# davidmhunt/mmwave_radar_processing

Hardware: AMD Instinct MI355X
Metric: radar frames/s on 256×128×12 ADC cube, 1/2/4/8 GPU; % HBM roofline (higher is better)
Workload: dtype f32; 1 GPU; IWR1843 synthetic 256x128x(4Rx x 3Tx) cube: Hann range FFT + Doppler FFT + 64-bin angle FFT -> complex64 [64,256,128] (BASELINE configs[1]); frames_per_gpu=1250, angle_bins=64, arch=gfx950:sramecc+:xnack-, compute_units=256

## Files before the change

mmwave_radar_processing_amd/csrc/mmw_cells64.h:

```cpp
#pragma once
#include "mmw_ctx.h"
#include "mmw_misc.h"
#include "mmw_bf16x3.h"

namespace mmw {

struct Cells64Args {
    const float2 *cubes;
    const int32_t *dets;
    const int32_t *counts;
    const int *flagpos;
    const int *n_flag;
    int dense_min;
    cplx<double> *out;
    int V, S, cap, n_ant, max_cells;
    AntList ants;
    const double *ws, *wc;
    const cplx<double> *twS, *twC;
};

constexpr int C64_NT = 512, C64_ROWS = 64, C64_PITCH = 137, C64_CELLS = 256, C64_ITEMS = 8 * C64_CELLS / C64_NT;
inline size_t cells64_lds(int S, int C, int) {
    return ((size_t)C64_ROWS * C64_PITCH + S) * 16 + ((size_t)S + C) * 8 + (size_t)C64_CELLS * 8 + 64;
}
inline int cells64_max_cells(int S, int C) {
    return C == 128 && cells64_lds(S, C, 0) <= 160 * 1024 - 512 ? C64_CELLS : 0;
}

template <int C>
__global__ __launch_bounds__(C64_NT) void k_cells64(Cells64Args a) {
    static_assert(C == 128, "one Doppler row = 8 lanes x 16 points");
    constexpr int P = C64_PITCH;
    extern __shared__ __attribute__((aligned(16))) char smem[];
    if (*a.n_flag < a.dense_min) return;
    const int S = a.S, tid = threadIdx.x, lane = tid & 63, wave = tid >> 6, n1 = tid & 7, rl = tid >> 3;
    cplx<double> *Z = reinterpret_cast<cplx<double> *>(smem);
    cplx<double> *twS = Z + C64_ROWS * P;
    double *wsl = reinterpret_cast<double *>(twS + S), *wcl = wsl + S;
    int *cell_rk = reinterpret_cast<int *>(wcl + C), *cell_e = cell_rk + C64_CELLS, *wcnt = cell_e + C64_CELLS;
    const long f = blockIdx.y;
    const int ai = blockIdx.x;
    int n_det = a.counts[f];
    if (n_det > a.cap) n_det = a.cap;
    if (n_det <= 0) return;
    for (int i = tid; i < S; i += C64_NT) {
        twS[i] = a.twS[i];
        wsl[i] = a.ws[i];
    }
    for (int i = tid; i < C; i += C64_NT) wcl[i] = a.wc[i];
    cplx<double> tw1[16];
#pragma unroll
    for (int k2 = 1; k2 < 16; ++k2) tw1[k2] = a.twC[(n1 * k2) & (C - 1)];
    const float2 *plane = a.cubes + (f * a.V + a.ants.idx[ai]) * (long)S * C;
    cplx<double> *slab = Z + rl * P;
    for (int c0 = 0;; c0 += C64_CELLS) {
        int running = 0;
        for (int det0 = 0; det0 < n_det; det0 += C64_NT) {
            const int det = det0 + tid;
            const int e = det < n_det ? a.flagpos[f * a.cap + det] - 1 : -1;
            const unsigned long long bal = __ballot(e >= 0);
            if (lane == 0) wcnt[wave] = __popcll(bal);
            __syncthreads();
            int before = running, total = running;
#pragma unroll
            for (int w = 0; w < C64_NT / 64; ++w) {
                const int cw = wcnt[w];
                if (w < wave) before += cw;
                total += cw;
            }
            const int ord = before + __popcll(bal & ((1ull << lane) - 1ull)) - c0;
            if (e >= 0 && ord >= 0 && ord < C64_CELLS) {
                const int r = a.dets[(f * a.cap + det) * 2];
                int k = a.dets[(f * a.cap + det) * 2 + 1] - C / 2;
                if (k < 0) k += C;
                cell_rk[ord] = (r << 16) | k;
                cell_e[ord] = e;
            }
            running = total;
            __syncthreads();
        }
        const int n_cells = running - c0 < C64_CELLS ? running - c0 : C64_CELLS;
        if (n_cells <= 0) break;
        cplx<double> acc[C64_ITEMS];
#pragma unroll
        for (int j = 0; j < C64_ITEMS; ++j) acc[j] = cplx<double>{0.0, 0.0};
        float2 raw[16];
        auto fetch = [&](int s0) {
            const int s = s0 + rl, sc = s < S ? s : S - 1;
            const float2 *rowp = plane + (long)sc * C;
#pragma unroll
            for (int n2 = 0; n2 < 16; ++n2) raw[n2] = rowp[n1 + 8 * n2];
        };
        fetch(0);
        for (int s0 = 0; s0 < S; s0 += C64_ROWS) {
            {
                const int s = s0 + rl;
                const double wrow = s < S ? wsl[s] : 0.0;
                cplx<double> x[16];
#pragma unroll
                for (int n2 = 0; n2 < 16; ++n2) {
                    const double w = wcl[n1 + 8 * n2] * wrow;
                    x[n2] = cplx<double>{(double)raw[n2].x * w, (double)raw[n2].y * w};
                }
                fetch(s0 + C64_ROWS < S ? s0 + C64_ROWS : s0);
                RegFFT<16, double>::run(x);
                static_for<16>([&](auto K) {
                    constexpr int k2 = decltype(K)::value;
                    const cplx<double> v = x[bitrev<16>(k2)];
                    slab[k2 * 8 + ((n1 + k2) & 7)] = k2 == 0 ? v : cmul(v, tw1[k2]);
                });
                __builtin_amdgcn_wave_barrier();
                cplx<double> ya[8], yb[8];
#pragma unroll
                for (int n = 0; n < 8; ++n) {
                    ya[n] = slab[n1 * 8 + ((n + n1) & 7)];
                    yb[n] = slab[(n1 + 8) * 8 + ((n + n1) & 7)];
                }
                RegFFT<8, double>::run(ya);
                RegFFT<8, double>::run(yb);
                __builtin_amdgcn_wave_barrier();
                static_for<8>([&](auto K) {
                    constexpr int k1 = decltype(K)::value;
                    slab[n1 + 16 * k1] = ya[bitrev<8>(k1)];
                    slab[n1 + 8 + 16 * k1] = yb[bitrev<8>(k1)];
                });
            }
            __syncthreads();
#pragma unroll
            for (int j = 0; j < C64_ITEMS; ++j) {
                const int it = tid + j * C64_NT, i = it >> 3, q = it & 7;
                if (i < n_cells) {
                    const int rk = cell_rk[i], r = rk >> 16, k = rk & 0xffff;
                    const int sq = s0 + 8 * q;
                    cplx<double> c = twS[(int)(((long)r * sq) % S)];
                    const cplx<double> step = twS[r % S];
                    const cplx<double> *zp = Z + (8 * q) * P + k;
                    cplx<double> sum = acc[j];
#pragma unroll
                    for (int t = 0; t < 8; ++t) {
                        const cplx<double> z = zp[t * P];
                        sum.x = fma(z.x, c.x, fma(-z.y, c.y, sum.x));
                        sum.y = fma(z.x, c.y, fma(z.y, c.x, sum.y));
                        c = cmul(c, step);
                    }
                    acc[j] = sum;
                }
            }
            __syncthreads();
        }
#pragma unroll
        for (int j = 0; j < C64_ITEMS; ++j) {
            const int it = tid + j * C64_NT, i = it >> 3, q = it & 7;
            cplx<double> s = acc[j];
            for (int d = 1; d < 8; d <<= 1) {
                s.x += __shfl_xor(s.x, d, 64);
                s.y += __shfl_xor(s.y, d, 64);
            }
            if (i < n_cells && q == 0) a.out[(long)cell_e[i] * a.n_ant + ai] = s;
        }
        if (running <= c0 + C64_CELLS) break;
        __syncthreads();
    }
}

struct Rd64Args {
    const float2 *cubes;
    long frame_stride;
    double *mag;
    cplx<double> *scratch;
    int n_frames;
    const double *ws, *wc;
    const cplx<double> *twS, *twC;
};
constexpr int R64_S = 256, R64_C = 128, R64_COLS = 32, R64_CP = 257;
inline size_t rd64_lds() { return (std::max((size_t)C64_ROWS * C64_PITCH, (size_t)R64_COLS * R64_CP) + R64_S + R64_C) * 16 + (R64_S + R64_C) * 8; }

__global__ __launch_bounds__(C64_NT) void k_rd_mag64_256x128(Rd64Args a) {
    constexpr int S = R64_S, C = R64_C, P = C64_PITCH;
    extern __shared__ __attribute__((aligned(16))) char smem[];
    const int tid = threadIdx.x;
    cplx<double> *Z = reinterpret_cast<cplx<double> *>(smem);
    cplx<double> *twl = Z + (C64_ROWS * P > R64_COLS * R64_CP ? C64_ROWS * P : R64_COLS * R64_CP);
    cplx<double> *twc = twl + S;
    double *wsl = reinterpret_cast<double *>(twc + C), *wcl = wsl + S;
    for (int i = tid; i < S; i += C64_NT) {
        wsl[i] = a.ws[i];
        twl[i] = a.twS[i];
    }
    for (int i = tid; i < C; i += C64_NT) {
        wcl[i] = a.wc[i];
        twc[i] = a.twC[i];
    }
    cplx<double> *T = a.scratch + (size_t)blockIdx.x * S * C;
    const auto t_rs = __builtin_amdgcn_make_buffer_rsrc(T, 0, S * C * 16, 0x00020000);
    __syncthreads();
    for (long f = blockIdx.x; f < a.n_frames; f += gridDim.x) {
        const float2 *plane = a.cubes + f * a.frame_stride;
        {
            const int n1 = tid & 7, rl = tid >> 3;
            cplx<double> *slab = Z + rl * P;
            float2 raw[16];
            auto fetch = [&](int s0) {
                const float2 *rowp = plane + (long)(s0 + rl) * C;
#pragma unroll
                for (int n2 = 0; n2 < 16; ++n2) raw[n2] = rowp[n1 + 8 * n2];
            };
            fetch(0);
            for (int s0 = 0; s0 < S; s0 += C64_ROWS) {
                const double wrow = wsl[s0 + rl];
                cplx<double> x[16];
#pragma unroll
                for (int n2 = 0; n2 < 16; ++n2) {
                    const double w = wcl[n1 + 8 * n2] * wrow;
                    x[n2] = cplx<double>{(double)raw[n2].x * w, (double)raw[n2].y * w};
                }
                fetch(s0 + C64_ROWS < S ? s0 + C64_ROWS : s0);
                RegFFT<16, double>::run(x);
                static_for<16>([&](auto K) {
                    constexpr int k2 = decltype(K)::value;
                    const cplx<double> v = x[bitrev<16>(k2)];
                    slab[k2 * 8 + ((n1 + k2) & 7)] = k2 == 0 ? v : cmul(v, twc[(n1 * k2) & (C - 1)]);
                });
                __builtin_amdgcn_wave_barrier();
                cplx<double> ya[8], yb[8];
#pragma unroll
                for (int n = 0; n < 8; ++n) {
                    ya[n] = slab[n1 * 8 + ((n + n1) & 7)];
                    yb[n] = slab[(n1 + 8) * 8 + ((n + n1) & 7)];
                }
                RegFFT<8, double>::run(ya);
                RegFFT<8, double>::run(yb);
                __builtin_amdgcn_wave_barrier();
                static_for<8>([&](auto K) {
                    constexpr int k1 = decltype(K)::value;
                    slab[n1 + 16 * k1] = ya[bitrev<8>(k1)];
                    slab[n1 + 8 + 16 * k1] = yb[bitrev<8>(k1)];
                });
                __syncthreads();
#pragma unroll 4
                for (int i = tid; i < C * C64_ROWS; i += C64_NT) {
                    const int k = i >> 6, r = i & 63;
                    T[k * S + s0 + r] = Z[r * P + k];
                }
                __syncthreads();
            }
        }
        asm volatile("s_waitcnt vmcnt(0)" ::: "memory");
        __syncthreads();
        {
            const int m1 = tid & 15, cl = tid >> 4;
            cplx<double> *slab = Z + cl * R64_CP;
            double *out = a.mag + f * (long)S * C;
            for (int k0 = 0; k0 < C; k0 += R64_COLS) {
                const int k = k0 + cl;
                cplx<double> x[16];
#pragma unroll
                for (int m2 = 0; m2 < 16; ++m2) {
                    const u32x4 v = __builtin_bit_cast(u32x4, __builtin_amdgcn_raw_buffer_load_b128(t_rs, (unsigned)((k * S + m1 + 16 * m2) * 16), 0, 1));
                    x[m2] = __builtin_bit_cast(cplx<double>, v);
                }
                RegFFT<16, double>::run(x);
                static_for<16>([&](auto Q) {
                    constexpr int q = decltype(Q)::value;
                    const cplx<double> v = x[bitrev<16>(q)];
                    slab[q * 16 + ((m1 + q) & 15)] = q == 0 ? v : cmul(v, twl[(m1 * q) & (S - 1)]);
                });
                __builtin_amdgcn_wave_barrier();
                cplx<double> y[16];
#pragma unroll
                for (int n = 0; n < 16; ++n) y[n] = slab[m1 * 16 + ((n + m1) & 15)];
                RegFFT<16, double>::run(y);
                int d = k + C / 2;
                if (d >= C) d -= C;
                static_for<16>([&](auto Pp) {
                    constexpr int p = decltype(Pp)::value;
                    const cplx<double> v = y[bitrev<16>(p)];
                    out[(long)(m1 + 16 * p) * C + d] = hypot(v.x, v.y);
                });
                __builtin_amdgcn_wave_barrier();
            }
        }
        __syncthreads();
    }
}

struct Argmax64ListArgs {
    const cplx<double> *cells;
    const int *n_flag, *list;
    int dense_min, dense_cap, n_ant, A, shift;
    int32_t *out_idx;
    const cplx<double> *twA;
};
__global__ __launch_bounds__(256) void k_argmax64_list(Argmax64ListArgs a) {
    int n = *a.n_flag;
    if (n < a.dense_min) return;
    if (n > a.dense_cap) n = a.dense_cap;
    const int lane = threadIdx.x & 63;
    for (int e = blockIdx.x * 4 + (threadIdx.x >> 6); e < n; e += gridDim.x * 4) {
        const int idx = argmax64_wave(a.cells + (long)e * a.n_ant, a.n_ant, a.A, a.shift, a.twA, lane);
        if (lane == 0) a.out_idx[a.list[e] & 0x7fffffff] = idx;
    }
}

}
```

mmwave_radar_processing_amd/csrc/mmw_cfar.h:

```cpp
#pragma once
#include "mmw_ctx.h"

namespace mmw {

template <int DEPTH, typename G> __device__ double np_pairwise(G get, int lo, int n) {
    if (n < 8) {
        double res = 0.0;
        for (int i = 0; i < n; ++i) res += get(lo + i);
        return res;
    }
    if (n <= 128 || DEPTH == 0) {
        double r0 = get(lo + 0), r1 = get(lo + 1), r2 = get(lo + 2), r3 = get(lo + 3);
        double r4 = get(lo + 4), r5 = get(lo + 5), r6 = get(lo + 6), r7 = get(lo + 7);
        int i = 8;
        for (; i < n - (n % 8); i += 8) {
            r0 += get(lo + i + 0); r1 += get(lo + i + 1); r2 += get(lo + i + 2); r3 += get(lo + i + 3);
            r4 += get(lo + i + 4); r5 += get(lo + i + 5); r6 += get(lo + i + 6); r7 += get(lo + i + 7);
        }
        double res = ((r0 + r1) + (r2 + r3)) + ((r4 + r5) + (r6 + r7));
        for (; i < n; ++i) res += get(lo + i);
        return res;
    }
    if constexpr (DEPTH > 0) {
        int n2 = n / 2;
// ... 567 lines not shown
    const double *base = tile + (ty * OSV_NV) * TW + tx;
#pragma unroll 1
    for (int y = 0; y < WR + OSV_NV - 1; ++y) {
        double v[WD];
#pragma unroll
        for (int wd = 0; wd < WD; ++wd) v[wd] = base[y * TW + wd];
        static_for<OSV_NV>([&](auto J) {
            constexpr int j = decltype(J)::value;
            const int wr = y - j;
            if (wr >= 0 && wr < WR) {
                if (wr >= TR && wr <= TR + 2 * GR) {
                    static_for<WD>([&](auto Wd) {
                        constexpr int wd = decltype(Wd)::value;
                        if constexpr (wd < TD || wd > TD + 2 * GD) below[j] += v[wd] < x[j] ? 1 : 0;
                    });
                } else {
#pragma unroll
                    for (int wd = 0; wd < WD; ++wd) below[j] += v[wd] < x[j] ? 1 : 0;
                }
            }
        });
    }
#pragma unroll
    for (int j = 0; j < OSV_NV; ++j) {
        const int r = rb + j;
        if (r >= p.R) break;
        const bool valid = r >= HR && r < p.R - HR && c >= HD && c < p.D - HD;
        p.mask[(long)blockIdx.z * plane + (long)r * p.D + c] = (valid && below[j] >= p.k_rank) ? 1 : 0;
    }
}

struct Cfar1dArgs {
    const double *x;
    double *thr, *noise;
    uint8_t *mask;
    int n_rows, L;
    int kind, T, G;
    double scale;
    int k_rank;
};

__device__ __forceinline__ double cfar1d_threshold(const Cfar1dArgs &p, const double *x, int i, double *est_out) {
    const int half = p.T + p.G;
    double thr = INFINITY, est = 0.0;
    if (i >= half && i < p.L - half) {
        const double *w = x + (i - half);
        const int rs = p.T + 2 * p.G + 1;
        if (p.kind == MMW_CFAR_CA) {
            double s = 0.0;
            if (p.L == 2 * half + 1) {
                s = np_pairwise<3>([&](int q) { return q < p.T ? w[q] : w[rs + q - p.T]; }, 0, 2 * p.T);
            } else {
                for (int q = 0; q < p.T; ++q) s += w[q];
                for (int q = 0; q < p.T; ++q) s += w[rs + q];
            }
            est = s / (double)(2 * p.T);
        } else if (p.kind == MMW_CFAR_OS) {
            est = kth_smallest([&](int q) { return q < p.T ? w[q] : w[rs + q - p.T]; }, 2 * p.T, p.k_rank);
        } else {
            const double ml = np_pairwise<2>([&](int q) { return w[q]; }, 0, p.T) / (double)p.T;
            const double mr = np_pairwise<2>([&](int q) { return w[rs + q]; }, 0, p.T) / (double)p.T;
            est = (ml != ml || mr != mr) ? ml + mr : (p.kind == MMW_CFAR_GO) ? fmax(ml, mr) : fmin(ml, mr);
        }
        thr = p.scale * est;
    }
    *est_out = est;
    return thr;
}

__global__ __launch_bounds__(256) void k_cfar1d(Cfar1dArgs p) {
    const long gid = (long)blockIdx.x * 256 + threadIdx.x;
    if (gid >= (long)p.n_rows * p.L) return;
    const int i = (int)(gid % p.L);
    const double *x = p.x + (gid - i);
    double est;
    const double thr = cfar1d_threshold(p, x, i, &est);
    if (p.thr) p.thr[gid] = thr;
    if (p.noise) p.noise[gid] = est;
    if (p.mask) p.mask[gid] = (x[i] > thr) ? 1 : 0;
}

__global__ __launch_bounds__(1024) void k_compact2d(const uint8_t *mask, int32_t *dets, int32_t *counts,
                                                    int R, int D, int cap) {
    __shared__ int wave_tot[16];
    __shared__ int wave_off[16];
    const long cells = (long)R * D;
    const uint8_t *m = mask + (long)blockIdx.x * cells;
    const int per = (int)((cells + 1023) / 1024);
    const long lo = (long)threadIdx.x * per;
    const long hi = lo + per < cells ? lo + per : cells;
    int cnt = 0;
    for (long i = lo; i < hi; ++i) cnt += m[i] ? 1 : 0;
    const int lane = threadIdx.x & 63, wave = threadIdx.x >> 6;
    int incl = cnt;
    for (int d = 1; d < 64; d <<= 1) {
        const int v = __shfl_up(incl, d, 64);
        if (lane >= d) incl += v;
    }
    if (lane == 63) wave_tot[wave] = incl;
    __syncthreads();
    if (threadIdx.x == 0) {
        int run = 0;
        for (int w = 0; w < 16; ++w) {
            wave_off[w] = run;
            run += wave_tot[w];
        }
        counts[blockIdx.x] = run;
    }
    __syncthreads();
    int pos = wave_off[wave] + incl - cnt;
    int32_t *out = dets + (long)blockIdx.x * cap * 2;
    for (long i = lo; i < hi; ++i) {
        if (m[i]) {
            if (pos < cap) {
                out[2 * pos] = (int32_t)(i / D);
                out[2 * pos + 1] = (int32_t)(i % D);
            }
            ++pos;
        }
    }
}

}
```

mmwave_radar_processing_amd/csrc/mmwgpu.hip:

```cpp
#include "mmw_ctx.h"
#include "mmw_launch.h"
#include "mmw_cfar.h"
#include "mmw_ground.h"
#include "mmw_seq.h"
#include "mmw_misc.h"
#include "mmw_czt.h"
#include "mmw_beamform.h"
#include "mmw_detect.h"
#include "mmw_cells64.h"

#include <algorithm>
#include <climits>
#include <chrono>
#include <memory>
#include <cstdlib>
#include <thread>

using namespace mmw;

namespace {

int env_int(const char *name, int dflt) {
    const char *s = std::getenv(name);
    return (s && *s) ? std::atoi(s) : dflt;
// ... 417 lines not shown
    MMW_REQUIRE(ctx && d_cubes && d_out, "null argument");
    MMW_REQUIRE(n_frames >= 0 && V > 0 && S > 0 && C > 0, "bad shape");
    if (n_frames == 0) return MMW_OK;
    {
        ProfScope ps(ctx, "rd");
        bool l1_done = false;
        const bool i16_folded = rv.i16 && rv.ntx > 1 &&
                                (fused_rd_runs(S, C) ||
                                 (rd_mixed_ct_supported(S, C) && !env_int("MMW_NO_MIXED_RD", 0)));
        if (rv.i16 && !i16_folded) {
            MMW_REQUIRE(rv.ntx >= 1 && rv.nrx >= 1, "int16 cubes are raw cubes");
            const long total = (long)n_frames * V * S * C;
            hipLaunchKernelGGL(k_reformat_i16, dim3((unsigned)((total + 255) / 256)), dim3(256), 0, ctx->stream,
                               (const short2 *)d_cubes, (float2 *)d_out, total, rv.nrx, rv.ntx, S, C);
            MMW_TRY(check_launch("reformat_i16"));
            d_cubes = d_out;
            rv = RawView{1, 0, rv.vskip, 0};
        }
        if (fused_rd_runs(S, C))
            MMW_TRY(launch_rd_fused(ctx, d_cubes, d_out, n_frames * V, S, C, rv, rv.ntx > 1 ? nullptr : d_l1, &l1_done));
        else if (rd_lds_supported(S, C) && !env_int("MMW_NO_FUSED_RD", 0) && !rd_mixed_ct_supported(S, C))
            MMW_TRY(launch_rd_lds(ctx, d_cubes, d_out, n_frames * V, S, C, rv));
        else if (rd_mixed_ct_supported(S, C) && !env_int("MMW_NO_MIXED_RD", 0)) {
            float *l1 = rv.ntx > 1 ? nullptr : d_l1;
            MMW_TRY(launch_rd_mixed_ct(ctx, d_cubes, (long)S * C, d_out, n_frames * V, S, C, rv, nullptr, 0, nullptr, false, l1));
            l1_done = l1 != nullptr;
        } else if (rd_mixed_supported(S, C) && !env_int("MMW_NO_MIXED_RD", 0))
            MMW_TRY((launch_rd_mixed<float, false>(ctx, d_cubes, (long)S * C, d_out, n_frames * V, S, C, rv)));
        else if (rv.ntx <= 1 && rd_split_ct_supported(S, C) && !env_int("MMW_NO_SPLIT_RD", 0))
            MMW_TRY(launch_rd_split_ct(ctx, d_cubes, d_out, n_frames * V, S, C, rv));
        else if (rv.ntx > 1) {
            const long total = (long)n_frames * V * S * C;
            hipLaunchKernelGGL(k_reformat, dim3((unsigned)((total + 255) / 256)), dim3(256), 0, ctx->stream,
                               (const float2 *)d_cubes, (float2 *)d_out, total, rv.nrx, rv.ntx, S, C);
            MMW_TRY(check_launch("reformat"));
            if (rd_split_ct_supported(S, C) && !env_int("MMW_NO_SPLIT_RD", 0))
                MMW_TRY(launch_rd_split_ct(ctx, d_out, d_out, n_frames * V, S, C, RawView{1, 0, rv.vskip}));
            else
                MMW_TRY(range_doppler_generic(ctx, d_out, d_out, n_frames, V, S, C));
        } else
            MMW_TRY(range_doppler_generic(ctx, d_cubes, d_out, n_frames, V, S, C));
        if (d_l1 && !l1_done) {
            MMW_REQUIRE(rv.ntx <= 1, "plane L1 norms are defined on virtual-array cubes");
            MMW_TRY(plane_l1_impl(ctx, d_cubes, d_l1, n_frames, V, S, C));
        }
    }
    if (d_mag_f32) MMW_TRY(abs_c64(ctx, d_out, (float *)d_mag_f32, (size_t)n_frames * V * S * C));
    return MMW_OK;
}

int mmw_range_doppler(mmw_ctx *ctx, const void *d_cubes, void *d_out, void *d_mag_f32, int n_frames, int V,
                      int S, int C) {
    MMW_REQUIRE(ctx, "ctx is null");
    MMW_JOIN(ctx);
    return range_doppler_impl(ctx, d_cubes, d_out, d_mag_f32, n_frames, V, S, C);
}

static int range_doppler_mag64_impl(mmw_ctx *ctx, const void *d_cubes, double *d_mag, int n_frames, int V, int S,
                                   int C, int rx_idx) {
    MMW_REQUIRE(ctx && d_cubes && d_mag, "null argument");
    MMW_REQUIRE(n_frames >= 0 && V > 0 && S > 0 && C > 0 && rx_idx >= 0 && rx_idx < V, "bad shape / rx_idx");
    if (n_frames == 0) return MMW_OK;
    ProfScope ps(ctx, "rd64");
    if (S == R64_S && C == R64_C && n_frames >= 8 && opt_int(ctx, "MMW_RD64_FUSED", 1)) {
        const int grid = std::min(n_frames, ctx->num_cu);
        MMW_TRY(ensure_scratch(ctx, (size_t)grid * S * C * sizeof(cplx<double>)));
        Rd64Args ra{};
        ra.cubes = (const float2 *)d_cubes + (long)rx_idx * S * C;
        ra.frame_stride = (long)V * S * C;
        ra.mag = d_mag;
        ra.scratch = (cplx<double> *)ctx->scratch;
        ra.n_frames = n_frames;
        const void *p;
        MMW_TRY(get_table<double>(ctx, TAB_HANN, S, &p));
        ra.ws = (const double *)p;
        MMW_TRY(get_table<double>(ctx, TAB_HANN, C, &p));
        ra.wc = (const double *)p;
        MMW_TRY(get_table<double>(ctx, TAB_TWIDDLE, S, &p));
        ra.twS = (const cplx<double> *)p;
        MMW_TRY(get_table<double>(ctx, TAB_TWIDDLE, C, &p));
        ra.twC = (const cplx<double> *)p;
        const size_t lds = rd64_lds();
        MMW_HIP(hipFuncSetAttribute(reinterpret_cast<const void *>(k_rd_mag64_256x128), hipFuncAttributeMaxDynamicSharedMemorySize, (int)lds));
        hipLaunchKernelGGL(k_rd_mag64_256x128, dim3((unsigned)grid), dim3(C64_NT), lds, ctx->stream, ra);
        return check_launch("rd_mag64_256x128");
    }
    RdMixedPlan mp;
    if (!is_pow2(S) || !is_pow2(C) || (long)S * C >= 8192)
        if (rd_mixed_plan(S, C, sizeof(cplx<double>), &mp) && !env_int("MMW_NO_MIXED_RD", 0))
            return launch_rd_mixed<double, true>(ctx, (const cplx<float> *)d_cubes + (long)rx_idx * S * C,
                                                 (long)V * S * C, d_mag, n_frames, S, C);
    const size_t plane_bytes = (size_t)S * C * sizeof(cplx<double>);
    long chunk = (long)(((size_t)128 << 20) / plane_bytes);
    if (chunk < 1) chunk = 1;
    if (chunk > n_frames) chunk = n_frames;
    MMW_TRY(ensure_scratch(ctx, (size_t)chunk * plane_bytes));
    FftArgs a{};
    a.out = ctx->scratch;
    a.inner = C;
    a.n_in = S;
    a.in_outer_stride = (long)V * S * C;
    a.out_outer_stride = (long)S * C;
    a.in_axis_stride = a.out_axis_stride = C;
    a.in_inner_stride = a.out_inner_stride = 1;
    MMW_TRY(get_table<double>(ctx, TAB_HANN, S, &a.win_axis));
    MMW_TRY(get_table<double>(ctx, TAB_HANN, C, &a.win_inner));
    a.scale = 1.0;
    FftArgs b{};
    b.in = ctx->scratch;
    b.inner = 1;
    b.n_in = C;
    b.in_outer_stride = b.out_outer_stride = C;
    b.in_axis_stride = b.out_axis_stride = 1;
    b.scale = 1.0;
    b.shift = 1;
    b.magnitude = 1;
    for (long f0 = 0; f0 < n_frames; f0 += chunk) {
        const int nf = (int)std::min<long>(chunk, n_frames - f0);
        a.in = (const cplx<float> *)d_cubes + (f0 * V + rx_idx) * (long)S * C;
        a.outer = nf;
        MMW_TRY((launch_fft_axis<double, float>(ctx, a, S, false)));
        b.out = d_mag + f0 * (long)S * C;
        b.outer = nf * S;
        MMW_TRY((launch_fft_axis<double, double>(ctx, b, C, true)));
    }
    return MMW_OK;
}

int mmw_range_doppler_mag64(mmw_ctx *ctx, const void *d_cubes, double *d_mag, int n_frames, int V, int S,
                            int C, int rx_idx) {
    MMW_REQUIRE(ctx, "ctx is null");
    MMW_JOIN(ctx);
    return range_doppler_mag64_impl(ctx, d_cubes, d_mag, n_frames, V, S, C, rx_idx);
}

static bool angle_fast_path(int V, long bins, int A, bool mag);

static int angle_fft_impl(mmw_ctx *ctx, const void *d_rd, void *d_out, int n_frames, int V, int S, int C, int A,
                         int flags) {
    MMW_REQUIRE(ctx && d_rd && d_out, "null argument");
    MMW_REQUIRE(n_frames >= 0 && V > 0 && S > 0 && C > 0 && A >= V, "bad shape (need A >= V)");
    MMW_REQUIRE((flags & ~7) == 0, "unknown flag bits %d", flags);
    if (n_frames == 0) return MMW_OK;
    const bool magnitude = flags & MMW_ANGLE_MAGNITUDE, window = !(flags & MMW_ANGLE_NO_WINDOW),
               shift = !(flags & MMW_ANGLE_NO_SHIFT);
    ProfScope ps(ctx, "angle");
    const long bins = (long)S * C;
    if (n_frames <= 65535 && angle_fast_path(V, bins, A, magnitude)) {
        float h[16];
        for (int i = 0; i < V; ++i) h[i] = window ? (float)np_window(TAB_HANN, i, V) : 1.f;
        switch (V) {
            case 4: return launch_angle64<4>(ctx, d_rd, d_out, n_frames, bins, magnitude, h, shift);
            case 8: return launch_angle64<8>(ctx, d_rd, d_out, n_frames, bins, magnitude, h, shift);
            case 12: return launch_angle64<12>(ctx, d_rd, d_out, n_frames, bins, magnitude, h, shift);
            default: return launch_angle64<16>(ctx, d_rd, d_out, n_frames, bins, magnitude, h, shift);
        }
    }
    FftArgs a{};
    a.in = d_rd;
    a.out = d_out;
    a.outer = n_frames;
    a.inner = (int)bins;
    a.n_in = V;
    a.in_outer_stride = (long)V * bins;
    a.out_outer_stride = (long)A * bins;
    a.in_axis_stride = a.out_axis_stride = bins;
    a.in_inner_stride = a.out_inner_stride = 1;
// ... 1098 lines not shown
    if (!no_mixed && rd_mixed_plan(S, C, sizeof(cplx<float>), &mp))
        return structured + mp.s1 + mp.s2 + mp.c1 + mp.c2 + 2 * (mp.rad_s[0] + mp.rad_s[1] + mp.rad_c[0] + mp.rad_c[1]);
    if (rd_split_ct_supported(S, C) && !env_int("MMW_NO_SPLIT_RD", 0)) return structured;
    int ulps = 8;
    for (int axis = 0; axis < 2; ++axis) {
        const int n = axis ? C : S;
        if (is_pow2(n)) ulps += 4 * ilog2(n);
        else ulps += n + 4;
    }
    return ulps;
}

static int launch_argmax_refine(mmw_ctx *ctx, const RefineArgs &ra) {
    const size_t lds = refine_tabs_lds(ra.S, ra.C);
    MMW_REQUIRE(lds <= 150 * 1024, "plane %d x %d too large for the refinement tables", ra.S, ra.C);
    if (lds > 48 * 1024) {
        MMW_HIP(hipFuncSetAttribute(reinterpret_cast<const void *>(k_argmax_refine_part), hipFuncAttributeMaxDynamicSharedMemorySize, (int)lds));
        MMW_HIP(hipFuncSetAttribute(reinterpret_cast<const void *>(k_argmax_refine_whole), hipFuncAttributeMaxDynamicSharedMemorySize, (int)lds));
    }
    if (ra.n_split > 0) {
        const int units = std::min(ra.n_split, std::max(1, 512));
        hipLaunchKernelGGL(k_argmax_refine_part, dim3(ra.parts, units), dim3(256), lds, ctx->stream, ra);
        MMW_TRY(check_launch("argmax_refine_part"));
        hipLaunchKernelGGL(k_argmax_refine_finish, dim3(std::min((ra.n_split + 3) / 4, ctx->num_cu)), dim3(256), 0, ctx->stream, ra);
        MMW_TRY(check_launch("argmax_refine_finish"));
    }
    if (ra.list_cap > ra.n_split) {
        hipLaunchKernelGGL(k_argmax_refine_whole, dim3(ctx->num_cu), dim3(256), lds, ctx->stream, ra);
        MMW_TRY(check_launch("argmax_refine_whole"));
    }
    return MMW_OK;
}

static int refine_parts(int n_frames) {
    int p = REFINE_PARTS;
    while (p > 2 && (long)p * n_frames > 60000) p /= 2;
    return p;
}

static int fill_refine_args(mmw_ctx *ctx, RefineArgs *ra, const void *d_cubes, const int32_t *d_dets, const int *n_flag, const int *list,
                            int list_cap, int n_split, cplx<double> *partial, int n_frames, int V, int S, int C, int cap, int A) {
    ra->cubes = (const float2 *)d_cubes, ra->dets = d_dets, ra->V = V, ra->cap = cap;
    ra->n_flag = n_flag, ra->list = list, ra->list_cap = list_cap;
    ra->partial = partial, ra->n_split = n_split, ra->parts = refine_parts(n_frames);
    const void *twA64, *twS64, *twC64, *ws64, *wc64;
    MMW_TRY(get_table<double>(ctx, TAB_TWIDDLE, A, &twA64));
    MMW_TRY(get_table<double>(ctx, TAB_TWIDDLE, S, &twS64));
    MMW_TRY(get_table<double>(ctx, TAB_TWIDDLE, C, &twC64));
    MMW_TRY(get_table<double>(ctx, TAB_HANN, S, &ws64));
    MMW_TRY(get_table<double>(ctx, TAB_HANN, C, &wc64));
    ra->S = S;
    ra->C = C;
    ra->A = A;
    ra->ws = (const double *)ws64;
    ra->wc = (const double *)wc64;
    ra->twS = (const cplx<double> *)twS64;
    ra->twC = (const cplx<double> *)twC64;
    ra->twA = (const cplx<double> *)twA64;
    return MMW_OK;
}

static float argmax_bound_div(const mmw_ctx *ctx) { return (float)std::max(1, opt_int(ctx, "MMW_ARGMAX_BOUND_DIV", 1)); }


int mmw_angle_argmax_exact(mmw_ctx *ctx, const void *d_cubes, const float *d_l1, const void *d_rd, const int32_t *d_dets,
                           const int32_t *d_counts, int32_t *d_idx, int n_frames, int V, int S, int C, int cap,
                           const int *h_ant, int n_ant, int A, int shift, int *h_n_refined) {
    MMW_REQUIRE(ctx && d_cubes && d_l1 && d_rd && d_dets && d_counts && d_idx, "null argument");
    MMW_JOIN(ctx);
    MMW_REQUIRE(n_frames >= 0 && n_frames <= 65535 && V > 0 && S > 0 && C > 0 && cap >= 0 && A > 0, "bad shape");
    MMW_REQUIRE((long)n_frames * cap < (1L << 31), "too many detection slots for one call");
    AntList ants{};
    MMW_TRY(fill_ant_list(h_ant, n_ant, V, A, &ants));
    if (h_n_refined) *h_n_refined = 0;
    if (n_frames == 0 || cap == 0) return MMW_OK;
    const void *twA = nullptr;
    MMW_TRY(get_table<float>(ctx, TAB_TWIDDLE, A, &twA));
    const int list_cap = n_frames * cap;
    const int n_split = std::min(list_cap, std::max(0, opt_int(ctx, "MMW_REFINE_SPLIT", 32768)));
    const int max_cells = C == 128 ? cells64_max_cells(S, C) : 0;
    const int dense_min = max_cells > 0 ? std::max(1, opt_int(ctx, "MMW_ARGMAX_DENSE_MIN", 8 * n_frames)) : 0;
    const int dense_cap = dense_min > 0 ? (int)std::min<long>(list_cap, 256L * n_frames) : 0;
    auto up = [](size_t b) { return (b + 255) & ~(size_t)255; };
    const size_t list_bytes = up(256 + (size_t)list_cap * sizeof(int));
    const size_t part_bytes = up((size_t)n_split * REFINE_PARTS * n_ant * sizeof(cplx<double>));
    const size_t pos_bytes = dense_min > 0 ? up((size_t)list_cap * sizeof(int)) : 0;
    const size_t cell_bytes = up((size_t)dense_cap * n_ant * sizeof(cplx<double>));
    MMW_TRY(ensure_scratch(ctx, list_bytes + part_bytes + pos_bytes + cell_bytes));
    int *d_nflag = (int *)ctx->scratch, *d_list = (int *)((char *)ctx->scratch + 256);
    int *d_flagpos = dense_min > 0 ? (int *)((char *)ctx->scratch + list_bytes + part_bytes) : nullptr;
    cplx<double> *d_cells = (cplx<double> *)((char *)ctx->scratch + list_bytes + part_bytes + pos_bytes);
    MMW_HIP(hipMemsetAsync(d_nflag, 0, 256, ctx->stream));
    if (d_flagpos) MMW_HIP(hipMemsetAsync(d_flagpos, 0, (size_t)list_cap * sizeof(int), ctx->stream));
    const float eps = 5.9604645e-8f, div = argmax_bound_div(ctx);
    ArgmaxRefine rf{d_l1, d_nflag, d_list, list_cap, (float)rd_error_ulps(S, C) * eps / div, 4.f * (float)(n_ant + 4) * eps / div,
                    d_flagpos, dense_cap};
    ProfScope ps(ctx, "argmax");
    dim3 grid(std::min((cap + 3) / 4, 32), n_frames);
    launch_angle_argmax(ctx, grid, (const float2 *)d_rd, d_dets, d_counts, d_idx, V, S, C, cap, ants, A, shift,
                        (const float2 *)twA, rf);
    MMW_TRY(check_launch("angle_argmax"));
    RefineArgs ra{};
    MMW_TRY(fill_refine_args(ctx, &ra, d_cubes, d_dets, d_nflag, d_list, list_cap, n_split, (cplx<double> *)((char *)ctx->scratch + list_bytes),
                             n_frames, V, S, C, cap, A));
    ra.out_idx = d_idx;
    ra.ants = ants;
    ra.shift = shift;
    ra.dense_min = dense_min;
    ra.dense_cap = dense_cap;
    if (dense_min > 0) {
        Cells64Args ca{};
        ca.cubes = (const float2 *)d_cubes;
        ca.dets = d_dets;
        ca.counts = d_counts;
        ca.flagpos = d_flagpos;
        ca.n_flag = d_nflag;
        ca.dense_min = dense_min;
        ca.out = d_cells;
        ca.V = V;
        ca.S = S;
        ca.cap = cap;
        ca.n_ant = n_ant;
        ca.max_cells = max_cells;
        ca.ants = ants;
        ca.ws = ra.ws;
        ca.wc = ra.wc;
        ca.twS = ra.twS;
        ca.twC = ra.twC;
        const size_t lds = cells64_lds(S, C, max_cells);
        MMW_HIP(hipFuncSetAttribute(reinterpret_cast<const void *>(k_cells64<128>), hipFuncAttributeMaxDynamicSharedMemorySize, (int)lds));
        hipLaunchKernelGGL(k_cells64<128>, dim3((unsigned)n_ant, (unsigned)n_frames), dim3(C64_NT), lds, ctx->stream, ca);
        MMW_TRY(check_launch("cells64"));
        Argmax64ListArgs la{d_cells, d_nflag, d_list, dense_min, dense_cap, n_ant, A, shift, d_idx, ra.twA};
        hipLaunchKernelGGL(k_argmax64_list, dim3((unsigned)std::min(std::max(dense_cap / 4, 1), 4 * ctx->num_cu)), dim3(256), 0, ctx->stream, la);
        MMW_TRY(check_launch("argmax64_list"));
    }
    MMW_TRY(launch_argmax_refine(ctx, ra));
    if (h_n_refined) {
        MMW_HIP(hipMemcpyAsync(h_n_refined, d_nflag, sizeof(int), hipMemcpyDeviceToHost, ctx->stream));
        MMW_HIP(hipStreamSynchronize(ctx->stream));
    }
    return MMW_OK;
}

static int ensure_det_queues(mmw_ctx *ctx, int rd_cus) {
    if (ctx->det_unavailable) return set_error(MMW_ERR_UNSUPPORTED, "detection queues unavailable on this runtime");
    if (ctx->q_drd && ctx->q_drd_cus == rd_cus) return MMW_OK;
    if (ctx->q_drd) {
        MMW_HIP(hipStreamSynchronize(ctx->q_drd));
        MMW_HIP(hipStreamSynchronize(ctx->q_dscr));
        MMW_HIP(hipStreamDestroy(ctx->q_drd));
        MMW_HIP(hipStreamDestroy(ctx->q_dscr));
        ctx->q_drd = ctx->q_dscr = nullptr;
    }
    if (!ctx->det_begin) {
        MMW_HIP(hipEventCreateWithFlags(&ctx->det_begin, hipEventDisableTiming));
        MMW_HIP(hipEventCreateWithFlags(&ctx->det_rd_done, hipEventDisableTiming));
        MMW_HIP(hipEventCreateWithFlags(&ctx->det_scr_done, hipEventDisableTiming));
    }
    const int words = (ctx->num_cu + 31) / 32;
    std::vector<uint32_t> m_rd(words, 0u), m_scr(words, 0u);
    for (int i = 0; i < ctx->num_cu; ++i) ((i < rd_cus) ? m_rd : m_scr)[i / 32] |= 1u << (i % 32);
    hipError_t e1 = hipExtStreamCreateWithCUMask(&ctx->q_drd, (uint32_t)words, m_rd.data()), e2 = hipSuccess;
    if (e1 == hipSuccess) e2 = hipExtStreamCreateWithCUMask(&ctx->q_dscr, (uint32_t)words, m_scr.data());
    if (e1 != hipSuccess || e2 != hipSuccess) {
        if (ctx->q_drd) (void)hipStreamDestroy(ctx->q_drd);
        ctx->q_drd = ctx->q_dscr = nullptr;
        ctx->det_unavailable = true;
        (void)hipGetLastError();
        return set_error(MMW_ERR_UNSUPPORTED, "detection queue creation failed: %s", hipGetErrorString(e1 != hipSuccess ? e1 : e2));
    }
    ctx->q_drd_cus = rd_cus;
    return MMW_OK;
}

namespace {
struct DetectPlan {
    bool ok, ct_window;
    int band_rows, band_pitch, words;
    size_t lds_screen, lds_cell;
};
DetectPlan detect_plan(int S, int C, int kind, int tr, int td, int gr, int gd, int n_az, int n_el, int A = 64) {
    DetectPlan p{};
    const long n = (long)S * C;
    const int hr = tr + gr, hd = td + gd;
    const int n_max = A == 64 ? DET_LATE_MAX_ANT : DET_MAX_ANT;
    if (kind != MMW_CFAR_CA || n_az > n_max || n_el > n_max || n > (1L << 20) || A < 1 || A > 1024) return p;
    p.words = (int)((n + 31) / 32);
    p.lds_cell = cell_exact_lds(S, C, 2 * hr + 1, 2 * hd + 1);
    if (p.lds_cell > 64 * 1024) return p;
    p.ct_window = with_cfar_window(tr, td, gr, gd, [](auto w) { return decltype(w)::compile_time; });
    p.band_pitch = p.ct_window ? det_band_pitch(C, hd) : C;
    const int unit = p.ct_window ? 4 : 1;
    const long cap_cells = (long)DET_LOADS * DET_NT * 2;
    int band = std::min<long>(std::max(1, tune_int("MMW_DETECT_BAND", DET_NT >= 1024 ? 32 : 24)), cap_cells / C - 2 * hr);
    band = std::min(band, std::max(unit, S - 2 * hr));
    band = band / unit * unit;
    if (band < unit) return p;
    p.band_rows = band;
    p.lds_screen = detect_screen_lds(band + 2 * hr, C, band, p.band_pitch, p.words, A);
    p.ok = p.lds_screen <= 160 * 1024 - 64;
    return p;
}
int fill_det_ant(const int *h_ant, int n_ant, int V, int A, DetAnt *out, AntList *full) {
    out->n = 0;
    full->n = 0;
    if (n_ant == 0) return MMW_OK;
    MMW_TRY(fill_ant_list(h_ant, n_ant, V, A, full));
    out->n = full->n;
    for (int i = 0; i < full->n && i < DET_LATE_MAX_ANT; ++i) out->idx[i] = full->idx[i];
    return MMW_OK;
}

struct DetectLayout {
    int cell_cap, list_cap, list_cap2;
// ... 563 lines not shown
```

Baseline: 275,700 frames/s.

## Shrink cells64 blocks for two-per-CU occupancy and vectorize CFAR compaction

The dense-cell kernel now uses 256-thread blocks with 32-row slabs and a smaller LDS footprint, so two blocks can share a CU. It loads input rows and window weights through buffer resources, splits accumulators into even and odd sets, and adds optional phase-clock instrumentation. The rd_mag kernel gets its own constants so it keeps its old shape. The CFAR compaction kernel is rewritten to scan 16-byte words with SWAR nonzero detection, a double-buffered prefetch and block-wide prefix sums in place of per-thread serial byte loops. Scratch layout is reordered so a single memset clears both the flag counter and the flag positions.

Measured after the change: 275,700 frames/s, median of 2. About the same (-0.0%).

```diff
diff --git a/mmwave_radar_processing_amd/csrc/mmw_cells64.h b/mmwave_radar_processing_amd/csrc/mmw_cells64.h
--- a/mmwave_radar_processing_amd/csrc/mmw_cells64.h
+++ b/mmwave_radar_processing_amd/csrc/mmw_cells64.h
@@ -17,18 +17,19 @@
     AntList ants;
     const double *ws, *wc;
     const cplx<double> *twS, *twC;
+    long long *clk;
 };
 
-constexpr int C64_NT = 512, C64_ROWS = 64, C64_PITCH = 137, C64_CELLS = 256, C64_ITEMS = 8 * C64_CELLS / C64_NT;
+constexpr int C64_NT = 256, C64_ROWS = 32, C64_PITCH = 129, C64_CELLS = 256, C64_ITEMS = 4 * C64_CELLS / C64_NT;
 inline size_t cells64_lds(int S, int C, int) {
-    return ((size_t)C64_ROWS * C64_PITCH + S) * 16 + ((size_t)S + C) * 8 + (size_t)C64_CELLS * 8 + 64;
+    return ((size_t)C64_ROWS * C64_PITCH + S) * 16 + (size_t)C * 8 + (size_t)C64_CELLS * 8 + 64;
 }
 inline int cells64_max_cells(int S, int C) {
     return C == 128 && cells64_lds(S, C, 0) <= 160 * 1024 - 512 ? C64_CELLS : 0;
 }
 
 template <int C>
-__global__ __launch_bounds__(C64_NT) void k_cells64(Cells64Args a) {
+__global__ __launch_bounds__(C64_NT, 2) void k_cells64(Cells64Args a) {
     static_assert(C == 128, "one Doppler row = 8 lanes x 16 points");
     constexpr int P = C64_PITCH;
     extern __shared__ __attribute__((aligned(16))) char smem[];
@@ -36,23 +37,29 @@
     const int S = a.S, tid = threadIdx.x, lane = tid & 63, wave = tid >> 6, n1 = tid & 7, rl = tid >> 3;
     cplx<double> *Z = reinterpret_cast<cplx<double> *>(smem);
     cplx<double> *twS = Z + C64_ROWS * P;
-    double *wsl = reinterpret_cast<double *>(twS + S), *wcl = wsl + S;
+    double *wcl = reinterpret_cast<double *>(twS + S);
     int *cell_rk = reinterpret_cast<int *>(wcl + C), *cell_e = cell_rk + C64_CELLS, *wcnt = cell_e + C64_CELLS;
     const long f = blockIdx.y;
     const int ai = blockIdx.x;
     int n_det = a.counts[f];
     if (n_det > a.cap) n_det = a.cap;
     if (n_det <= 0) return;
-    for (int i = tid; i < S; i += C64_NT) {
-        twS[i] = a.twS[i];
-        wsl[i] = a.ws[i];
-    }
+    for (int i = tid; i < S; i += C64_NT) twS[i] = a.twS[i];
     for (int i = tid; i < C; i += C64_NT) wcl[i] = a.wc[i];
     cplx<double> tw1[16];
 #pragma unroll
     for (int k2 = 1; k2 < 16; ++k2) tw1[k2] = a.twC[(n1 * k2) & (C - 1)];
     const float2 *plane = a.cubes + (f * a.V + a.ants.idx[ai]) * (long)S * C;
     cplx<double> *slab = Z + rl * P;
+    const bool timed = a.clk && blockIdx.y == gridDim.y / 2 && blockIdx.x == 0 && tid == 0;
+    long long ph[6] = {0, 0, 0, 0, 0, 0}, t_prev = 0;
+    auto mark = [&](int i) {
+        if (a.clk) {
+            const long long t = (long long)__builtin_amdgcn_s_memtime();
+            if (i >= 0) ph[i] += t - t_prev;
+            t_prev = t;
+        }
+    };
     for (int c0 = 0;; c0 += C64_CELLS) {
         int running = 0;
         for (int det0 = 0; det0 < n_det; det0 += C64_NT) {
@@ -81,21 +88,28 @@
         }
         const int n_cells = running - c0 < C64_CELLS ? running - c0 : C64_CELLS;
         if (n_cells <= 0) break;
-        cplx<double> acc[C64_ITEMS];
-#pragma unroll
-        for (int j = 0; j < C64_ITEMS; ++j) acc[j] = cplx<double>{0.0, 0.0};
+        cplx<double> acc_e[C64_ITEMS], acc_o[C64_ITEMS];
+#pragma unroll
+        for (int j = 0; j < C64_ITEMS; ++j) acc_e[j] = acc_o[j] = cplx<double>{0.0, 0.0};
         float2 raw[16];
+        double wrow_next;
+        const auto ws_rs = __builtin_amdgcn_make_buffer_rsrc(const_cast<double *>(a.ws), 0, S * 8, 0x00020000);
+        const auto plane_rs = __builtin_amdgcn_make_buffer_rsrc(const_cast<float2 *>(plane), 0, S * C * 8, 0x00020000);
         auto fetch = [&](int s0) {
             const int s = s0 + rl, sc = s < S ? s : S - 1;
-            const float2 *rowp = plane + (long)sc * C;
-#pragma unroll
-            for (int n2 = 0; n2 < 16; ++n2) raw[n2] = rowp[n1 + 8 * n2];
+            const unsigned row0 = (unsigned)(sc * C + n1) * 8u;
+#pragma unroll
+            for (int n2 = 0; n2 < 16; ++n2)
+                raw[n2] = __builtin_bit_cast(float2, __builtin_amdgcn_raw_buffer_load_b64(plane_rs, row0 + 64u * n2, 0, 0));
+            wrow_next = __builtin_bit_cast(double, __builtin_amdgcn_raw_buffer_load_b64(ws_rs, (unsigned)sc * 8u, 0, 0));
         };
         fetch(0);
         for (int s0 = 0; s0 < S; s0 += C64_ROWS) {
             {
-                const int s = s0 + rl;
-                const double wrow = s < S ? wsl[s] : 0.0;
+                mark(-1);
+                if (a.clk) asm volatile("s_waitcnt vmcnt(0)" ::: "memory");
+                mark(0);
+                const double wrow = s0 + rl < S ? wrow_next : 0.0;
                 cplx<double> x[16];
 #pragma unroll
                 for (int n2 = 0; n2 < 16; ++n2) {
@@ -125,42 +139,55 @@
                     slab[n1 + 8 + 16 * k1] = yb[bitrev<8>(k1)];
                 });
             }
+            mark(1);
             __syncthreads();
-#pragma unroll
-            for (int j = 0; j < C64_ITEMS; ++j) {
-                const int it = tid + j * C64_NT, i = it >> 3, q = it & 7;
-                if (i < n_cells) {
-                    const int rk = cell_rk[i], r = rk >> 16, k = rk & 0xffff;
-                    const int sq = s0 + 8 * q;
-                    cplx<double> c = twS[(int)(((long)r * sq) % S)];
-                    const cplx<double> step = twS[r % S];
-                    const cplx<double> *zp = Z + (8 * q) * P + k;
-                    cplx<double> sum = acc[j];
-#pragma unroll
-                    for (int t = 0; t < 8; ++t) {
-                        const cplx<double> z = zp[t * P];
-                        sum.x = fma(z.x, c.x, fma(-z.y, c.y, sum.x));
-                        sum.y = fma(z.x, c.y, fma(z.y, c.x, sum.y));
-                        c = cmul(c, step);
+            mark(2);
+            auto sums = [&](cplx<double> (&acc)[C64_ITEMS]) {
+#pragma unroll
+                for (int j = 0; j < C64_ITEMS; ++j) {
+                    const int it = tid + j * C64_NT, i = it >> 2, q = it & 3;
+                    if (i < n_cells) {
+                        const int rk = cell_rk[i], r = rk >> 16, k = rk & 0xffff;
+                        const int sq = s0 + 8 * q;
+                        cplx<double> c = twS[(int)(((long)r * sq) % S)];
+                        const cplx<double> step = twS[r % S];
+                        const cplx<double> *zp = Z + (8 * q) * P + k;
+                        cplx<double> sum = acc[j];
+#pragma unroll
+                        for (int t = 0; t < 8; ++t) {
+                            const cplx<double> z = zp[t * P];
+                            sum.x = fma(z.x, c.x, fma(-z.y, c.y, sum.x));
+                            sum.y = fma(z.x, c.y, fma(z.y, c.x, sum.y));
+                            c = cmul(c, step);
+                        }
+                        acc[j] = sum;
                     }
-                    acc[j] = sum;
-                }
-            }
+                }
+            };
+            if (s0 & C64_ROWS) sums(acc_o);
+            else sums(acc_e);
+            mark(3);
             __syncthreads();
+            mark(4);
+            ++ph[5];
         }
 #pragma unroll
         for (int j = 0; j < C64_ITEMS; ++j) {
-            const int it = tid + j * C64_NT, i = it >> 3, q = it & 7;
-            cplx<double> s = acc[j];
-            for (int d = 1; d < 8; d <<= 1) {
-                s.x += __shfl_xor(s.x, d, 64);
-                s.y += __shfl_xor(s.y, d, 64);
-            }
-            if (i < n_cells && q == 0) a.out[(long)cell_e[i] * a.n_ant + ai] = s;
+            const int it = tid + j * C64_NT, i = it >> 2, q = it & 3;
+            cplx<double> se = acc_e[j], so = acc_o[j];
+            for (int d = 1; d < 4; d <<= 1) {
+                se.x += __shfl_xor(se.x, d, 64);
+                se.y += __shfl_xor(se.y, d, 64);
+                so.x += __shfl_xor(so.x, d, 64);
+                so.y += __shfl_xor(so.y, d, 64);
+            }
+            if (i < n_cells && q == 0) a.out[(long)cell_e[i] * a.n_ant + ai] = cplx<double>{se.x + so.x, se.y + so.y};
         }
         if (running <= c0 + C64_CELLS) break;
         __syncthreads();
     }
+    if (timed)
+        for (int i = 0; i < 6; ++i) a.clk[i] = ph[i];
 }
 
 struct Rd64Args {
@@ -172,22 +199,22 @@
     const double *ws, *wc;
     const cplx<double> *twS, *twC;
 };
-constexpr int R64_S = 256, R64_C = 128, R64_COLS = 32, R64_CP = 257;
-inline size_t rd64_lds() { return (std::max((size_t)C64_ROWS * C64_PITCH, (size_t)R64_COLS * R64_CP) + R64_S + R64_C) * 16 + (R64_S + R64_C) * 8; }
-
-__global__ __launch_bounds__(C64_NT) void k_rd_mag64_256x128(Rd64Args a) {
-    constexpr int S = R64_S, C = R64_C, P = C64_PITCH;
+constexpr int R64_S = 256, R64_C = 128, R64_COLS = 32, R64_CP = 257, R64_NT = 512, R64_ROWS = 64, R64_PITCH = 137;
+inline size_t rd64_lds() { return (std::max((size_t)R64_ROWS * R64_PITCH, (size_t)R64_COLS * R64_CP) + R64_S + R64_C) * 16 + (R64_S + R64_C) * 8; }
+
+__global__ __launch_bounds__(R64_NT) void k_rd_mag64_256x128(Rd64Args a) {
+    constexpr int S = R64_S, C = R64_C, P = R64_PITCH;
     extern __shared__ __attribute__((aligned(16))) char smem[];
     const int tid = threadIdx.x;
     cplx<double> *Z = reinterpret_cast<cplx<double> *>(smem);
-    cplx<double> *twl = Z + (C64_ROWS * P > R64_COLS * R64_CP ? C64_ROWS * P : R64_COLS * R64_CP);
+    cplx<double> *twl = Z + (R64_ROWS * P > R64_COLS * R64_CP ? R64_ROWS * P : R64_COLS * R64_CP);
     cplx<double> *twc = twl + S;
     double *wsl = reinterpret_cast<double *>(twc + C), *wcl = wsl + S;
-    for (int i = tid; i < S; i += C64_NT) {
+    for (int i = tid; i < S; i += R64_NT) {
         wsl[i] = a.ws[i];
         twl[i] = a.twS[i];
     }
-    for (int i = tid; i < C; i += C64_NT) {
+    for (int i = tid; i < C; i += R64_NT) {
         wcl[i] = a.wc[i];
         twc[i] = a.twC[i];
     }
@@ -206,7 +233,7 @@
                 for (int n2 = 0; n2 < 16; ++n2) raw[n2] = rowp[n1 + 8 * n2];
             };
             fetch(0);
-            for (int s0 = 0; s0 < S; s0 += C64_ROWS) {
+            for (int s0 = 0; s0 < S; s0 += R64_ROWS) {
                 const double wrow = wsl[s0 + rl];
                 cplx<double> x[16];
 #pragma unroll
@@ -214,7 +241,7 @@
                     const double w = wcl[n1 + 8 * n2] * wrow;
                     x[n2] = cplx<double>{(double)raw[n2].x * w, (double)raw[n2].y * w};
                 }
-                fetch(s0 + C64_ROWS < S ? s0 + C64_ROWS : s0);
+                fetch(s0 + R64_ROWS < S ? s0 + R64_ROWS : s0);
                 RegFFT<16, double>::run(x);
                 static_for<16>([&](auto K) {
                     constexpr int k2 = decltype(K)::value;
@@ -238,7 +265,7 @@
                 });
                 __syncthreads();
 #pragma unroll 4
-                for (int i = tid; i < C * C64_ROWS; i += C64_NT) {
+                for (int i = tid; i < C * R64_ROWS; i += R64_NT) {
                     const int k = i >> 6, r = i & 63;
                     T[k * S + s0 + r] = Z[r * P + k];
                 }
diff --git a/mmwave_radar_processing_amd/csrc/mmw_cfar.h b/mmwave_radar_processing_amd/csrc/mmw_cfar.h
--- a/mmwave_radar_processing_amd/csrc/mmw_cfar.h
+++ b/mmwave_radar_processing_amd/csrc/mmw_cfar.h
@@ -673,43 +673,69 @@
 
 __global__ __launch_bounds__(1024) void k_compact2d(const uint8_t *mask, int32_t *dets, int32_t *counts,
                                                     int R, int D, int cap) {
-    __shared__ int wave_tot[16];
-    __shared__ int wave_off[16];
+    __shared__ int wave_tot[2][16];
     const long cells = (long)R * D;
     const uint8_t *m = mask + (long)blockIdx.x * cells;
-    const int per = (int)((cells + 1023) / 1024);
-    const long lo = (long)threadIdx.x * per;
-    const long hi = lo + per < cells ? lo + per : cells;
-    int cnt = 0;
-    for (long i = lo; i < hi; ++i) cnt += m[i] ? 1 : 0;
+    const long head = (long)(reinterpret_cast<uintptr_t>(m) & 15);
+    const long n_words = (head + cells + 15) >> 4;
     const int lane = threadIdx.x & 63, wave = threadIdx.x >> 6;
-    int incl = cnt;
-    for (int d = 1; d < 64; d <<= 1) {
-        const int v = __shfl_up(incl, d, 64);
-        if (lane >= d) incl += v;
-    }
-    if (lane == 63) wave_tot[wave] = incl;
-    __syncthreads();
-    if (threadIdx.x == 0) {
-        int run = 0;
-        for (int w = 0; w < 16; ++w) {
-            wave_off[w] = run;
-            run += wave_tot[w];
-        }
-        counts[blockIdx.x] = run;
-    }
-    __syncthreads();
-    int pos = wave_off[wave] + incl - cnt;
     int32_t *out = dets + (long)blockIdx.x * cap * 2;
-    for (long i = lo; i < hi; ++i) {
-        if (m[i]) {
-            if (pos < cap) {
-                out[2 * pos] = (int32_t)(i / D);
-                out[2 * pos + 1] = (int32_t)(i % D);
-            }
-            ++pos;
-        }
-    }
-}
-
-}
+    auto load = [&](long w, unsigned (&v)[4]) {
+        v[0] = v[1] = v[2] = v[3] = 0u;
+        if (w >= n_words) return;
+        const long i0 = w * 16 - head;
+        if (i0 >= 0 && i0 + 16 <= cells) {
+            const uint4 q = *reinterpret_cast<const uint4 *>(m + i0);
+            v[0] = q.x, v[1] = q.y, v[2] = q.z, v[3] = q.w;
+        } else {
+            for (int j = 0; j < 16; ++j)
+                if (i0 + j >= 0 && i0 + j < cells) v[j >> 2] |= (unsigned)m[i0 + j] << (8 * (j & 3));
+        }
+    };
+    unsigned cur[4], nxt[4];
+    load(threadIdx.x, cur);
+    int base = 0, buf = 0;
+    for (long w0 = 0; w0 < n_words; w0 += 1024, buf ^= 1) {
+        load(w0 + 1024 + threadIdx.x, nxt);
+        unsigned nz[4];
+        int cnt = 0;
+#pragma unroll
+        for (int d = 0; d < 4; ++d) {
+            nz[d] = (((cur[d] & 0x7f7f7f7fu) + 0x7f7f7f7fu) | cur[d]) & 0x80808080u;
+            cnt += __popc(nz[d]);
+        }
+        int incl = cnt;
+        for (int d = 1; d < 64; d <<= 1) {
+            const int v = __shfl_up(incl, d, 64);
+            if (lane >= d) incl += v;
+        }
+        if (lane == 63) wave_tot[buf][wave] = incl;
+        __syncthreads();
+        int pos = base + incl - cnt;
+#pragma unroll
+        for (int v = 0; v < 16; ++v) {
+            const int t = wave_tot[buf][v];
+            if (v < wave) pos += t;
+            base += t;
+        }
+        if (cnt) {
+            const long i0 = (w0 + threadIdx.x) * 16 - head;
+#pragma unroll
+            for (int d = 0; d < 4; ++d) {
+                for (unsigned bits = nz[d]; bits; bits &= bits - 1) {
+                    if (pos < cap) {
+                        const long i = i0 + 4 * d + ((__ffs((int)bits) - 1) >> 3);
+                        out[2 * pos] = (int32_t)(i / D);
+                        out[2 * pos + 1] = (int32_t)(i % D);
+                    }
+                    ++pos;
+                }
+            }
+        }
+#pragma unroll
+        for (int d = 0; d < 4; ++d) cur[d] = nxt[d];
+    }
+    if (threadIdx.x == 0) counts[blockIdx.x] = base;
+}
+
+}
diff --git a/mmwave_radar_processing_amd/csrc/mmwgpu.hip b/mmwave_radar_processing_amd/csrc/mmwgpu.hip
--- a/mmwave_radar_processing_amd/csrc/mmwgpu.hip
+++ b/mmwave_radar_processing_amd/csrc/mmwgpu.hip
@@ -523,7 +523,7 @@
         ra.twC = (const cplx<double> *)p;
         const size_t lds = rd64_lds();
         MMW_HIP(hipFuncSetAttribute(reinterpret_cast<const void *>(k_rd_mag64_256x128), hipFuncAttributeMaxDynamicSharedMemorySize, (int)lds));
-        hipLaunchKernelGGL(k_rd_mag64_256x128, dim3((unsigned)grid), dim3(C64_NT), lds, ctx->stream, ra);
+        hipLaunchKernelGGL(k_rd_mag64_256x128, dim3((unsigned)grid), dim3(R64_NT), lds, ctx->stream, ra);
         return check_launch("rd_mag64_256x128");
     }
     RdMixedPlan mp;
@@ -1788,16 +1788,17 @@
     const int dense_min = max_cells > 0 ? std::max(1, opt_int(ctx, "MMW_ARGMAX_DENSE_MIN", 8 * n_frames)) : 0;
     const int dense_cap = dense_min > 0 ? (int)std::min<long>(list_cap, 256L * n_frames) : 0;
     auto up = [](size_t b) { return (b + 255) & ~(size_t)255; };
-    const size_t list_bytes = up(256 + (size_t)list_cap * sizeof(int));
+    const size_t pos_bytes = dense_min > 0 ? up((size_t)list_cap * sizeof(int)) : 0;
+    const size_t list_bytes = up((size_t)list_cap * sizeof(int));
     const size_t part_bytes = up((size_t)n_split * REFINE_PARTS * n_ant * sizeof(cplx<double>));
-    const size_t pos_bytes = dense_min > 0 ? up((size_t)list_cap * sizeof(int)) : 0;
     const size_t cell_bytes = up((size_t)dense_cap * n_ant * sizeof(cplx<double>));
-    MMW_TRY(ensure_scratch(ctx, list_bytes + part_bytes + pos_bytes + cell_bytes));
-    int *d_nflag = (int *)ctx->scratch, *d_list = (int *)((char *)ctx->scratch + 256);
-    int *d_flagpos = dense_min > 0 ? (int *)((char *)ctx->scratch + list_bytes + part_bytes) : nullptr;
-    cplx<double> *d_cells = (cplx<double> *)((char *)ctx->scratch + list_bytes + part_bytes + pos_bytes);
-    MMW_HIP(hipMemsetAsync(d_nflag, 0, 256, ctx->stream));
-    if (d_flagpos) MMW_HIP(hipMemsetAsync(d_flagpos, 0, (size_t)list_cap * sizeof(int), ctx->stream));
+    MMW_TRY(ensure_scratch(ctx, 256 + pos_bytes + list_bytes + part_bytes + cell_bytes));
+    char *base = (char *)ctx->scratch;
+    int *d_nflag = (int *)base, *d_flagpos = dense_min > 0 ? (int *)(base + 256) : nullptr;
+    int *d_list = (int *)(base + 256 + pos_bytes);
+    cplx<double> *d_part = (cplx<double> *)(base + 256 + pos_bytes + list_bytes);
+    cplx<double> *d_cells = (cplx<double> *)(base + 256 + pos_bytes + list_bytes + part_bytes);
+    MMW_HIP(hipMemsetAsync(d_nflag, 0, 256 + (d_flagpos ? (size_t)list_cap * sizeof(int) : 0), ctx->stream));
     const float eps = 5.9604645e-8f, div = argmax_bound_div(ctx);
     ArgmaxRefine rf{d_l1, d_nflag, d_list, list_cap, (float)rd_error_ulps(S, C) * eps / div, 4.f * (float)(n_ant + 4) * eps / div,
                     d_flagpos, dense_cap};
@@ -1807,7 +1808,7 @@
                         (const float2 *)twA, rf);
     MMW_TRY(check_launch("angle_argmax"));
     RefineArgs ra{};
-    MMW_TRY(fill_refine_args(ctx, &ra, d_cubes, d_dets, d_nflag, d_list, list_cap, n_split, (cplx<double> *)((char *)ctx->scratch + list_bytes),
+    MMW_TRY(fill_refine_args(ctx, &ra, d_cubes, d_dets, d_nflag, d_list, list_cap, n_split, d_part,
                              n_frames, V, S, C, cap, A));
     ra.out_idx = d_idx;
     ra.ants = ants;
@@ -1833,10 +1834,20 @@
         ca.wc = ra.wc;
         ca.twS = ra.twS;
         ca.twC = ra.twC;
+        PhaseClocks clk;
+        if (opt_int(ctx, "MMW_PHASE_CLOCKS", 0)) MMW_TRY(clk.alloc(6, ctx->stream));
+        ca.clk = clk.d;
         const size_t lds = cells64_lds(S, C, max_cells);
         MMW_HIP(hipFuncSetAttribute(reinterpret_cast<const void *>(k_cells64<128>), hipFuncAttributeMaxDynamicSharedMemorySize, (int)lds));
         hipLaunchKernelGGL(k_cells64<128>, dim3((unsigned)n_ant, (unsigned)n_frames), dim3(C64_NT), lds, ctx->stream, ca);
         MMW_TRY(check_launch("cells64"));
+        if (clk.d) {
+            long long h[6] = {0};
+            MMW_TRY(clk.fetch(h, 6, ctx->stream));
+            std::fprintf(stderr, "cells64 %dx%d, %d antennas: %lld passes; clocks per pass: load wait %lld fft+exchange %lld barrier %lld "
+                         "cell sums %lld barrier %lld\n", S, C, n_ant, h[5], h[0] / std::max(1LL, h[5]), h[1] / std::max(1LL, h[5]),
+                         h[2] / std::max(1LL, h[5]), h[3] / std::max(1LL, h[5]), h[4] / std::max(1LL, h[5]));
+        }
         Argmax64ListArgs la{d_cells, d_nflag, d_list, dense_min, dense_cap, n_ant, A, shift, d_idx, ra.twA};
         hipLaunchKernelGGL(k_argmax64_list, dim3((unsigned)std::min(std::max(dense_cap / 4, 1), 4 * ctx->num_cu)), dim3(256), 0, ctx->stream, la);
         MMW_TRY(check_launch("argmax64_list"));
```
